# jamornsriwasansak/evplp

Measured on AMD Instinct MI355X. Metric: Mpaths/s, higher is better.
Workload: dtype f32

## Files before the change

evplp_amd/csrc/device_common.hpp:

```cpp
#pragma once
#include "evplp_types.h"
#include "ev_math.h"

namespace evplp {

#define EV_PI 3.14159265358979323846f
#define EV_INV_PI 0.318309886183790671537767526745028724068919291480912897495f
#define EV_DEV __device__ __forceinline__

struct V3 { float x, y, z; };
EV_DEV V3 v3(float x, float y, float z) { V3 r; r.x = x; r.y = y; r.z = z; return r; }
EV_DEV V3 v3(const float *p) { return v3(p[0], p[1], p[2]); }
EV_DEV V3 v3(float4 a) { return v3(a.x, a.y, a.z); }
EV_DEV V3 operator+(V3 a, V3 b) { return v3(a.x + b.x, a.y + b.y, a.z + b.z); }
EV_DEV V3 operator-(V3 a, V3 b) { return v3(a.x - b.x, a.y - b.y, a.z - b.z); }
EV_DEV V3 operator-(V3 a) { return v3(-a.x, -a.y, -a.z); }
EV_DEV V3 operator*(V3 a, V3 b) { return v3(a.x * b.x, a.y * b.y, a.z * b.z); }
EV_DEV V3 operator*(V3 a, float s) { return v3(a.x * s, a.y * s, a.z * s); }
EV_DEV V3 operator/(V3 a, float s) { return v3(a.x / s, a.y / s, a.z / s); }
EV_DEV float dot(V3 a, V3 b) { return a.x * b.x + a.y * b.y + a.z * b.z; }
EV_DEV V3 cross(V3 a, V3 b) { return v3(a.y * b.z - a.z * b.y, a.z * b.x - a.x * b.z, a.x * b.y - a.y * b.x); }
EV_DEV V3 normalize(V3 v) { float inv = 1.0f / sqrtf(dot(v, v)); return v * inv; }
EV_DEV V3 reflect(V3 i, V3 n) { float d = dot(n, i); return i - (n * 2.0f) * d; }
EV_DEV V3 faceforward(V3 n, V3 i, V3 nref) { return n * copysignf(1.0f, dot(i, nref)); }
// ... 203 lines not shown
    V3 p = v3(sin_t * cp, sin_t * sp, cos_t);
    Onb o = onb_make(r);
    out = onb_inverse(o, p);
    float unsafe_cos = dot(out, normal);
    float cos_n = fmaxf(unsafe_cos, 0.f);
    float cos_r = fmaxf(dot(out, r), 0.f);
    if (unsafe_cos > 0.0f) pdfw = (e + 1.0f) * 0.5f * evm_powf(cos_r, e) * EV_INV_PI;
    else pdfw = 0.0f;
    return rho_s * ((e + 2.0f) / (e + 1.0f) * cos_n);
}

EV_DEV V3 light_sample(const SceneDev &sc, V3 &position, V3 &normal, float &pdf, Rng &rng) {
    float r = rng_uniform(rng);
    uint32_t count = (uint32_t)sc.light_count, first = 0;
    while (count > 0) {
        uint32_t it = first, step = count / 2; it += step;
        if (sc.light_cdf[it] < r) { first = ++it; count -= step + 1; } else count = step;
    }
    if (first >= (uint32_t)sc.light_count) first = (uint32_t)sc.light_count - 1;
    const TriAttr &ta = sc.attrs[sc.light_first + (int32_t)first];
    float x = rng_uniform(rng);
    float y = rng_uniform(rng);
    float sq = sqrtf(x), beta = sq * (1.0f - y), gamma = sq * y;
    V3 p1 = v3(ta.v), p2 = v3(ta.v + 3), p3 = v3(ta.v + 6);
    position = p1 * beta + p2 * gamma + p3 * (1.0f - gamma - beta);
    normal = normalize(cross(p2 - p1, p3 - p1));
    pdf = 1.f / sc.light_area;
    return v3(sc.light_intensity) * sc.light_area;
}

EV_DEV bool slab_hit(const float *lo, const float *hi, V3 inv, V3 noi, float tmin, float tmax) {
    float t0x = __builtin_fmaf(lo[0], inv.x, noi.x), t1x = __builtin_fmaf(hi[0], inv.x, noi.x);
    float t0y = __builtin_fmaf(lo[1], inv.y, noi.y), t1y = __builtin_fmaf(hi[1], inv.y, noi.y);
    float t0z = __builtin_fmaf(lo[2], inv.z, noi.z), t1z = __builtin_fmaf(hi[2], inv.z, noi.z);
    float tn = fmaxf(fmaxf(fminf(t0x, t1x), fminf(t0y, t1y)), fmaxf(fminf(t0z, t1z), tmin));
    float tf = fminf(fminf(fmaxf(t0x, t1x), fmaxf(t0y, t1y)), fminf(fmaxf(t0z, t1z), tmax));
    return tn <= tf;
}
EV_DEV float slab_near(const float *lo, const float *hi, V3 inv, V3 noi, float tmin, float tmax, bool &hit) {
    float t0x = __builtin_fmaf(lo[0], inv.x, noi.x), t1x = __builtin_fmaf(hi[0], inv.x, noi.x);
    float t0y = __builtin_fmaf(lo[1], inv.y, noi.y), t1y = __builtin_fmaf(hi[1], inv.y, noi.y);
    float t0z = __builtin_fmaf(lo[2], inv.z, noi.z), t1z = __builtin_fmaf(hi[2], inv.z, noi.z);
    float tn = fmaxf(fmaxf(fminf(t0x, t1x), fminf(t0y, t1y)), fmaxf(fminf(t0z, t1z), tmin));
    float tf = fminf(fminf(fmaxf(t0x, t1x), fmaxf(t0y, t1y)), fminf(fmaxf(t0z, t1z), tmax));
    hit = tn <= tf;
    return tn;
}
EV_DEV float safe_rcp(float d) {
    float a = fabsf(d) < 1e-30f ? copysignf(1e-30f, d) : d;
    return __builtin_amdgcn_rcpf(a);
}

typedef int v16i __attribute__((ext_vector_type(16)));
typedef int v8i __attribute__((ext_vector_type(8)));
EV_DEV v16i sload16(const void *base, uint32_t byte_offset) {
    v16i r;
    asm("s_load_dwordx16 %0, %1, %2\n\ts_waitcnt lgkmcnt(0)" : "=&s"(r) : "s"(base), "s"(byte_offset));
    return r;
}
EV_DEV v8i sload8(const void *base, uint32_t byte_offset) {
    v8i r;
    asm("s_load_dwordx8 %0, %1, %2\n\ts_waitcnt lgkmcnt(0)" : "=&s"(r) : "s"(base), "s"(byte_offset));
    return r;
}
EV_DEV void sload16x2(const void *base, uint32_t byte_offset, v16i &a, v16i &b) {
    asm("s_load_dwordx16 %0, %2, %3\n\ts_load_dwordx16 %1, %2, %3 offset:0x40\n\ts_waitcnt lgkmcnt(0)" : "=&s"(a), "=&s"(b) : "s"(base), "s"(byte_offset));
}
EV_DEV void sload16x3(const void *base, uint32_t byte_offset, v16i &a, v16i &b, v16i &c) {
    asm("s_load_dwordx16 %0, %3, %4\n\ts_load_dwordx16 %1, %3, %4 offset:0x40\n\ts_load_dwordx16 %2, %3, %4 offset:0x80\n\ts_waitcnt lgkmcnt(0)"
        : "=&s"(a), "=&s"(b), "=&s"(c) : "s"(base), "s"(byte_offset));
}
template <class T> EV_DEV const T *pinned(const T *p) { asm("" : "+s"(p)); return p; }
#ifndef EVPLP_RING_NT
#define EVPLP_RING_NT 1
#endif
EV_DEV void lds_dma16(const void *gsrc, uint32_t lds_dst) {
    unsigned keep;
#if EVPLP_RING_NT
    asm volatile("s_mov_b32 %0, m0\n\ts_mov_b32 m0, %2\n\ts_nop 0\n\tglobal_load_lds_dwordx4 %1, off nt\n\ts_mov_b32 m0, %0" : "=&s"(keep) : "v"(gsrc), "s"(lds_dst) : "memory");
#else
    asm volatile("s_mov_b32 %0, m0\n\ts_mov_b32 m0, %2\n\ts_nop 0\n\tglobal_load_lds_dwordx4 %1, off\n\ts_mov_b32 m0, %0" : "=&s"(keep) : "v"(gsrc), "s"(lds_dst) : "memory");
#endif
}
EV_DEV void wait_vmcnt0() { asm volatile("s_waitcnt vmcnt(0)" ::: "memory"); }
template <int N> EV_DEV void wait_vmcnt() { asm volatile("s_waitcnt vmcnt(%0)" ::"n"(N) : "memory"); }
template <class T> EV_DEV uint32_t lds_offset(const T *p) { return (uint32_t)(uintptr_t)p; }
EV_DEV float f_of(int x) { return __int_as_float(x); }
EV_DEV v2f pk(int a, int b) { v2f r; r.x = __int_as_float(a); r.y = __int_as_float(b); return r; }
EV_DEV v2f bc(float a) { v2f r; r.x = a; r.y = a; return r; }
EV_DEV v2f pk_fma(v2f a, v2f b, v2f c) { return __builtin_elementwise_fma(a, b, c); }
EV_DEV v2f pk_min(v2f a, v2f b) { return __builtin_elementwise_min(a, b); }
EV_DEV v2f pk_max(v2f a, v2f b) { return __builtin_elementwise_max(a, b); }

EV_DEV v2f rcp_exact2(v2f x) {
#pragma clang fp contract(off)
    v2f r; r.x = __builtin_amdgcn_rcpf(x.x); r.y = __builtin_amdgcn_rcpf(x.y);
    const v2f one = bc(1.0f);
    const v2f e = pk_fma(-x, r, one);
    r = pk_fma(e, r, r);
    const v2f err = pk_fma(-x, r, one);
    return pk_fma(err, r, r);
}
EV_DEV unsigned long long ballot64(bool p) { return __builtin_amdgcn_ballot_w64(p); }
struct Hit2 { bool a, b; };
EV_DEV Hit2 tri_pair_test(v2f p0x, v2f p0y, v2f p0z, v2f e0x, v2f e0y, v2f e0z, v2f e1x, v2f e1y, v2f e1z, v2f nx, v2f ny, v2f nz,
                          V3 o, V3 d, float tmin, float tmax) {
#pragma clang fp contract(off)
    const v2f dx = bc(d.x), dy = bc(d.y), dz = bc(d.z);
    v2f den = pk_fma(nz, dz, pk_fma(ny, dy, nx * dx));
    const v2f inv = rcp_exact2(den);
    v2f qx = (p0x - bc(o.x)) * inv, qy = (p0y - bc(o.y)) * inv, qz = (p0z - bc(o.z)) * inv;
    v2f ix = pk_fma(dy, qz, -(dz * qy)), iy = pk_fma(dz, qx, -(dx * qz)), iz = pk_fma(dx, qy, -(dy * qx));
    v2f beta = pk_fma(iz, e1z, pk_fma(iy, e1y, ix * e1x));
    v2f gamma = pk_fma(iz, e0z, pk_fma(iy, e0y, ix * e0x));
    v2f t = pk_fma(nz, qz, pk_fma(ny, qy, nx * qx));
    const v2f rest = bc(1.0f) - (beta + gamma);
    Hit2 h;
    h.a = (t.x < tmax) & (t.x > tmin) & (__builtin_fminf(__builtin_fminf(beta.x, gamma.x), rest.x) >= 0.0f);
    h.b = (t.y < tmax) & (t.y > tmin) & (__builtin_fminf(__builtin_fminf(beta.y, gamma.y), rest.y) >= 0.0f);
    return h;
}

struct PairOps { v2f p0x, p0y, p0z, e0x, e0y, e0z, e1x, e1y, e1z, nx, ny, nz; };
EV_DEV bool tri_pair_any(const PairOps &T, V3 o, V3 d, float tmin, float tmax, uint32_t *exact_runs = nullptr) {
    if (exact_runs) (*exact_runs)++;
    Hit2 h = tri_pair_test(T.p0x, T.p0y, T.p0z, T.e0x, T.e0y, T.e0z, T.e1x, T.e1y, T.e1z, T.nx, T.ny, T.nz, o, d, tmin, tmax);
    return h.a | h.b;
}
struct LeafOps { PairOps A, B; uint32_t cnt; };
EV_DEV LeafOps fetch_leaf(const char *leaf_base, uint32_t leafref) {
    const uint32_t id = ~leafref;
    LeafOps L; L.cnt = (id & 3u) + 1u;
    const uint32_t off = (id >> 2) * 192u;
    v16i a, b;
    if (L.cnt > 2u) {
        v16i c;
        sload16x3(leaf_base, off, a, b, c);
        L.B.p0x = pk(b[8], b[9]); L.B.p0y = pk(b[10], b[11]); L.B.p0z = pk(b[12], b[13]); L.B.e0x = pk(b[14], b[15]); L.B.e0y = pk(c[0], c[1]); L.B.e0z = pk(c[2], c[3]);
        L.B.e1x = pk(c[4], c[5]); L.B.e1y = pk(c[6], c[7]); L.B.e1z = pk(c[8], c[9]); L.B.nx = pk(c[10], c[11]); L.B.ny = pk(c[12], c[13]); L.B.nz = pk(c[14], c[15]);
    } else sload16x2(leaf_base, off, a, b);
    L.A.p0x = pk(a[0], a[1]); L.A.p0y = pk(a[2], a[3]); L.A.p0z = pk(a[4], a[5]); L.A.e0x = pk(a[6], a[7]); L.A.e0y = pk(a[8], a[9]); L.A.e0z = pk(a[10], a[11]);
    L.A.e1x = pk(a[12], a[13]); L.A.e1y = pk(a[14], a[15]); L.A.e1z = pk(b[0], b[1]); L.A.nx = pk(b[2], b[3]); L.A.ny = pk(b[4], b[5]); L.A.nz = pk(b[6], b[7]);
    return L;
}

EV_DEV PairOps fetch_leaf_a(const char *leaf_base, uint32_t off, v16i &b) {
    v16i a;
    sload16x2(leaf_base, off, a, b);
    PairOps A;
    A.p0x = pk(a[0], a[1]); A.p0y = pk(a[2], a[3]); A.p0z = pk(a[4], a[5]); A.e0x = pk(a[6], a[7]); A.e0y = pk(a[8], a[9]); A.e0z = pk(a[10], a[11]);
    A.e1x = pk(a[12], a[13]); A.e1y = pk(a[14], a[15]); A.e1z = pk(b[0], b[1]); A.nx = pk(b[2], b[3]); A.ny = pk(b[4], b[5]); A.nz = pk(b[6], b[7]);
    return A;
}
EV_DEV PairOps fetch_leaf_b(const char *leaf_base, uint32_t off, const v16i &b) {
    const v16i c = sload16(leaf_base, off + 128u);
    PairOps B;
    B.p0x = pk(b[8], b[9]); B.p0y = pk(b[10], b[11]); B.p0z = pk(b[12], b[13]); B.e0x = pk(b[14], b[15]); B.e0y = pk(c[0], c[1]); B.e0z = pk(c[2], c[3]);
    B.e1x = pk(c[4], c[5]); B.e1y = pk(c[6], c[7]); B.e1z = pk(c[8], c[9]); B.nx = pk(c[10], c[11]); B.ny = pk(c[12], c[13]); B.nz = pk(c[14], c[15]);
    return B;
}

EV_DEV int lane_write(int value, int slot, int old) { return ((int)(threadIdx.x & 63u) == slot) ? value : old; }
EV_DEV int lane_read(int v, int slot) { return __builtin_amdgcn_readlane(v, slot); }

EV_DEV float clamp01(float x) { return __builtin_amdgcn_fmed3f(x, 0.0f, 1.0f); }

#ifndef EVPLP_TRAVERSAL_STATS
#define EVPLP_TRAVERSAL_STATS 0
#endif
struct WalkStats { uint32_t nodes, leaves, pairs, exact; int32_t hit_leaf; uint32_t syn; };

#ifndef EVPLP_WALK_ASM
#define EVPLP_WALK_ASM 1
#endif
#define EV_WALK_VISIT_ASM(T0, T1, T2, T3, T4, T5, T0L, T0H, T1L, T1H, T2L, T2H, T3L, T3H, T4L, T4H, T5L, T5H) EV_WALK_VISIT_ASM_("s", T0, T1, T2, T3, T4, T5, T0L, T0H, T1L, T1H, T2L, T2H, T3L, T3H, T4L, T4H, T5L, T5H)
#define EV_WALK_VISIT_ASM_(NC, T0, T1, T2, T3, T4, T5, T0L, T0H, T1L, T1H, T2L, T2H, T3L, T3H, T4L, T4H, T5L, T5H)                               \
    asm volatile(                                                                                                                            \
        "v_pk_fma_f32 " T0 ", %[cx], %[pa], %[pd] op_sel:[0,0,0] op_sel_hi:[1,0,0]\n\t"                                                                                     \
        "v_pk_fma_f32 " T1 ", %[cy], %[pa], %[pd] op_sel:[0,1,1] op_sel_hi:[1,1,1]\n\t"                                                                                     \
        "v_pk_fma_f32 " T2 ", %[cz], %[pb], %[pe] op_sel:[0,0,0] op_sel_hi:[1,0,0]\n\t"                                                                                     \
        "v_pk_fma_f32 " T3 ", %[hx], %[pb], " T0 " op_sel:[0,1,0] op_sel_hi:[1,1,1] neg_lo:[0,1,0] neg_hi:[0,1,0]\n\t"                                                        \
        "v_pk_fma_f32 " T4 ", %[hy], %[pc], " T1 " op_sel:[0,0,0] op_sel_hi:[1,0,1] neg_lo:[0,1,0] neg_hi:[0,1,0]\n\t"                                                        \
        "v_pk_fma_f32 " T5 ", %[hz], %[pc], " T2 " op_sel:[0,1,0] op_sel_hi:[1,1,1] neg_lo:[0,1,0] neg_hi:[0,1,0]\n\t"                                                        \
        "v_pk_fma_f32 " T0 ", %[hx], %[pb], " T0 " op_sel:[0,1,0] op_sel_hi:[1,1,1]\n\t"                                                                                     \
        "v_pk_fma_f32 " T1 ", %[hy], %[pc], " T1 " op_sel:[0,0,0] op_sel_hi:[1,0,1]\n\t"                                                                                     \
        "v_pk_fma_f32 " T2 ", %[hz], %[pc], " T2 " op_sel:[0,1,0] op_sel_hi:[1,1,1]\n\t"                                                                                     \
        "v_max3_f32 " T3L ", " T3L ", " T4L ", " T5L " clamp\n\t"                                                                            \
        "v_min3_f32 " T0L ", " T0L ", " T1L ", " T2L " clamp\n\t"                                                                            \
        "v_max3_f32 " T3H ", " T3H ", " T4H ", " T5H " clamp\n\t"                                                                            \
        "v_min3_f32 " T0H ", " T0H ", " T1H ", " T2H " clamp\n\t"                                                                            \
        "v_cmp_lt_f32 vcc, " T3L ", " T0L "\n\t"                                                                                             \
        "v_cmp_lt_f32 %[m1], " T3H ", " T0H "\n\t"                                                                                           \
        "s_or_b64 %[t64], vcc, %[m1]\n\t"                                                                                                    \
        "s_cbranch_scc0 L_pop%=\n\t"                                                                                                         \
        "s_cmp_eq_u64 vcc, 0\n\t"                                                                                                            \
        "s_cbranch_scc1 L_c1%=\n\t"                                                                                                          \
        "s_cmp_eq_u64 %[m1], 0\n\t"                                                                                                          \
        "s_cbranch_scc1 L_c0%=\n\t"                                                                                                          \
        "s_bcnt1_i32_b64 %[p0], vcc\n\t"                                                                                                     \
        "s_bcnt1_i32_b64 %[p1], %[m1]\n\t"                                                                                                   \
        "s_cmp_ge_i32 %[p0], %[p1]\n\t"                                                                                                      \
        "s_cselect_b32 %[p0], %[c1], %[c0]\n\t"                                                                                              \
        "s_cselect_b32 %[cur], %[c0], %[c1]\n\t"                                                                                             \
        "s_mov_b32 m0, %[sp]\n\t"                                                                                                            \
        "s_add_i32 %[sp], %[sp], 1\n\t"                                                                                                      \
        "v_writelane_b32 %[vstack], %[p0], m0\n\t"                                                                                           \
        "s_branch L_end%=\n"                                                                                                                 \
        "L_c0%=:\n\t"                                                                                                                        \
        "s_mov_b32 %[cur], %[c0]\n\t"                                                                                                        \
        "s_branch L_end%=\n"                                                                                                                 \
        "L_c1%=:\n\t"                                                                                                                        \
        "s_mov_b32 %[cur], %[c1]\n\t"                                                                                                        \
        "s_branch L_end%=\n"                                                                                                                 \
        "L_pop%=:\n\t"                                                                                                                       \
        "s_brev_b32 %[cur], 1\n\t"                                                                                                           \
        "s_cmp_eq_u32 %[sp], 0\n\t"                                                                                                          \
        "s_cbranch_scc1 L_end%=\n\t"                                                                                                         \
        "s_sub_i32 %[sp], %[sp], 1\n\t"                                                                                                      \
        "s_nop 0\n\t"                                                                                                                        \
        "v_readlane_b32 %[cur], %[vstack], %[sp]\n"                                                                                          \
        "L_end%=:\n"                                                                                                                         \
        : [cur] "+s"(cur), [sp] "+s"(sp), [vstack] "+v"(vstack), [m1] "=&s"(m1_), [t64] "=&s"(t64_), [p0] "=&s"(p0_), [p1] "=&s"(p1_)          \
        : [cx] NC(cx_), [cy] NC(cy_), [cz] NC(cz_), [hx] NC(hx_), [hy] NC(hy_), [hz] NC(hz_), [c0] "s"(c0_), [c1] "s"(c1_),              \
          [pa] "v"(pa_), [pb] "v"(pb_), [pc] "v"(pc_),                                     \
          [pd] "v"(pd_), [pe] "v"(pe_), [lane] "v"(lane_id)                                                                 \
        : "vcc", "scc", "m0", T0L, T0H, T1L, T1H, T2L, T2H, T3L, T3H, T4L, T4H, T5L, T5H)

template <int VT = 0, bool CUT = false>
EV_DEV bool occluded_wave(const char *node_base, const char *leaf_base, V3 o, V3 d, float tmin, float tmax, bool alive_lane, WalkStats *ws = nullptr, const char *cut = nullptr, uint32_t cut_off = 0u,
                          const float4 *cut_lds = nullptr) {
    unsigned long long alive = ballot64(alive_lane), hitm = 0ull;
    if (alive == 0ull) return false;
    uint32_t cut_end = 0u;
    constexpr bool kCutLds = CUT && VT != 0 && EVPLP_WALK_ASM && !EVPLP_TRAVERSAL_STATS;
    if constexpr (kCutLds) {
        const int32_t nsyn = __builtin_amdgcn_readfirstlane(__float_as_int(cut_lds[3].z));
        if (nsyn == 0) return false;
        cut_off = 0u; cut_end = (uint32_t)nsyn;
    } else if constexpr (CUT) {
        int32_t nsyn;
        asm volatile("s_load_dword %0, %1, %2 offset:0x38\n\ts_waitcnt lgkmcnt(0)" : "=s"(nsyn) : "s"(cut), "s"(cut_off) : "memory");
        if (nsyn == 0) return false;
        cut_end = cut_off + ((uint32_t)nsyn << 6);
    }
    const V3 inv0 = v3(safe_rcp(d.x), safe_rcp(d.y), safe_rcp(d.z));
    const float ku = 1.0f / (tmax - tmin);
    const V3 inv = inv0 * ku;
    const v2f ivx = bc(inv.x), ivy = bc(inv.y), ivz = bc(inv.z);
    const v2f avx = bc(fabsf(inv.x)), avy = bc(fabsf(inv.y)), avz = bc(fabsf(inv.z));
    const float dead = __builtin_inff();
    v2f nox = bc(alive_lane ? (-(o.x * inv0.x) - tmin) * ku : dead), noy = bc(alive_lane ? (-(o.y * inv0.y) - tmin) * ku : dead),
        noz = bc(alive_lane ? (-(o.z * inv0.z) - tmin) * ku : dead);
    int sp = 0;
    int vstack = 0;
    int32_t cur = 0;
#if EVPLP_WALK_ASM && !EVPLP_TRAVERSAL_STATS
    if constexpr (VT != 0) {
        static_assert(VT == 52 || VT == 116, "reserved temporaries: v[52:63] or v[116:127]");
        const int lane_id = (int)(threadIdx.x & 63u);
        v2f pa_, pb_, pc_, pd_, pe_;
        pa_.x = ivx.x; pa_.y = ivy.x; pb_.x = ivz.x; pb_.y = avx.x; pc_.x = avy.x; pc_.y = avz.x;
        pd_.x = nox.x; pd_.y = noy.x; pe_.x = noz.x; pe_.y = noz.x;
#define EV_VISIT(N)                                                                                                                          \
        {                                                                                                                                    \
            const v2f cx_ = pk(N[0], N[1]), cy_ = pk(N[2], N[3]), cz_ = pk(N[4], N[5]), hx_ = pk(N[6], N[7]), hy_ = pk(N[8], N[9]), hz_ = pk(N[10], N[11]); \
            const int32_t c0_ = N[12], c1_ = N[13];                                                                                          \
            unsigned long long m1_, t64_; int32_t p0_, p1_;                                                                                  \
            if constexpr (VT == 52) EV_WALK_VISIT_ASM("v[52:53]", "v[54:55]", "v[56:57]", "v[58:59]", "v[60:61]", "v[62:63]", "v52", "v53", "v54", "v55", "v56", "v57", "v58", "v59", "v60", "v61", "v62", "v63"); \
            else EV_WALK_VISIT_ASM("v[116:117]", "v[118:119]", "v[120:121]", "v[122:123]", "v[124:125]", "v[126:127]", "v116", "v117", "v118", "v119", "v120", "v121", "v122", "v123", "v124", "v125", "v126", "v127"); \
        }
        for (;;) {
            if constexpr (CUT) {
                if (cut_off >= cut_end) break;
                v16i syn;
                {
                    const float4 *q = cut_lds + 4u * cut_off;
#pragma unroll
                    for (int w = 0; w < 4; w++) {
                        const float4 qq = q[w];
                        if (w < 3 || true) { syn[4 * w] = __builtin_amdgcn_readfirstlane(__float_as_int(qq.x)); syn[4 * w + 1] = __builtin_amdgcn_readfirstlane(__float_as_int(qq.y)); }
                        if (w < 3) { syn[4 * w + 2] = __builtin_amdgcn_readfirstlane(__float_as_int(qq.z)); syn[4 * w + 3] = __builtin_amdgcn_readfirstlane(__float_as_int(qq.w)); }
                    }
                    syn[14] = 0; syn[15] = 0;
                }
                cut_off++;
                EV_VISIT(syn)
            }
            for (;;) {
                while (cur >= 0) {
                    const v16i n = sload16(node_base, (uint32_t)cur << 6);
                    EV_VISIT(n)
                }
                if (cur == kNoChild) break;
                const uint32_t cnt = (((uint32_t)~cur) & 3u) + 1u, loff = (((uint32_t)~cur) >> 2) * 192u;
                bool any;
                if constexpr (CUT) {
                    v16i lb;
                    { const PairOps A = fetch_leaf_a(leaf_base, loff, lb); any = tri_pair_any(A, o, d, tmin, tmax); }
                    if (cnt > 2u) { const PairOps B = fetch_leaf_b(leaf_base, loff, lb); any = any | tri_pair_any(B, o, d, tmin, tmax); }
                } else {
                    const LeafOps L = fetch_leaf(leaf_base, (uint32_t)cur);
                    any = tri_pair_any(L.A, o, d, tmin, tmax);
                    if (cnt > 2u) any = any | tri_pair_any(L.B, o, d, tmin, tmax);
                }
                const unsigned long long hm = ballot64(any) & alive;
                if (hm != 0ull) {
                    hitm |= hm;
                    alive &= ~hm;
                    if (alive == 0ull) return ((hitm >> (threadIdx.x & 63u)) & 1ull) != 0ull;
                    if (any) { pd_ = bc(dead); pe_ = bc(dead); }
                }
                if (sp == 0) break;
                sp--;
                cur = lane_read(vstack, sp);
            }
            if constexpr (!CUT) break;
        }
#undef EV_VISIT
        return ((hitm >> (threadIdx.x & 63u)) & 1ull) != 0ull;
    }
#endif
    auto visit_cpp = [&](const v16i &n) {
        const v2f ax = pk_fma(pk(n[0], n[1]), ivx, nox), ay = pk_fma(pk(n[2], n[3]), ivy, noy), az = pk_fma(pk(n[4], n[5]), ivz, noz);
        const v2f hx = pk(n[6], n[7]), hy = pk(n[8], n[9]), hz = pk(n[10], n[11]);
        const v2f enx = pk_fma(hx, -avx, ax), eny = pk_fma(hy, -avy, ay), enz = pk_fma(hz, -avz, az);
        const v2f exx = pk_fma(hx, avx, ax), exy = pk_fma(hy, avy, ay), exz = pk_fma(hz, avz, az);
        const float tn0 = clamp01(fmaxf(fmaxf(enx.x, eny.x), enz.x)), tf0 = clamp01(fminf(fminf(exx.x, exy.x), exz.x));
        const float tn1 = clamp01(fmaxf(fmaxf(enx.y, eny.y), enz.y)), tf1 = clamp01(fminf(fminf(exx.y, exy.y), exz.y));
        const unsigned long long m0 = ballot64(tn0 < tf0), m1 = ballot64(tn1 < tf1);
        const int32_t c0 = n[12], c1 = n[13];
        const uint32_t a0 = (uint32_t)m0 | (uint32_t)(m0 >> 32), a1 = (uint32_t)m1 | (uint32_t)(m1 >> 32);
        if ((a0 | a1) == 0u) { if (sp == 0) cur = kNoChild; else { sp--; cur = lane_read(vstack, sp); } return; }
        if (a0 == 0u) { cur = c1; return; }
        if (a1 == 0u) { cur = c0; return; }
        int p0, p1;
        asm("s_bcnt1_i32_b64 %0, %1" : "=s"(p0) : "s"(m0) : "scc");
        asm("s_bcnt1_i32_b64 %0, %1" : "=s"(p1) : "s"(m1) : "scc");
        const bool first0 = p0 >= p1;
        const int32_t oth = first0 ? c1 : c0;
        vstack = lane_write(oth, sp, vstack);
        sp++;
        cur = first0 ? c0 : c1;
    };
    for (;;) {
        if constexpr (CUT) {
            if (cut_off >= cut_end) break;
            const v16i syn = sload16(cut, cut_off);
            cut_off += 64u;
#if EVPLP_TRAVERSAL_STATS
            if (ws) { ws->nodes++; ws->syn++; }
#endif
            visit_cpp(syn);
        }
        for (;;) {
            while (cur >= 0) {
                const v16i n = sload16(node_base, (uint32_t)cur << 6);
#if EVPLP_TRAVERSAL_STATS
                if (ws) ws->nodes++;
#endif
                visit_cpp(n);
            }
            if (cur == kNoChild) break;
            {
                const uint32_t id = (uint32_t)~cur;
                const uint32_t cnt = (id & 3u) + 1u;
                const LeafOps L = fetch_leaf(leaf_base, (uint32_t)cur);
#if EVPLP_TRAVERSAL_STATS
                if (ws) { ws->leaves++; ws->pairs += cnt > 2u ? 2u : 1u; }
                uint32_t *ex = ws ? &ws->exact : nullptr;
// ... 374 lines not shown
```

evplp_amd/csrc/kernels_gather.hip:

```cpp
#include "device_common.hpp"
#include "kernels.h"
#include <algorithm>

namespace evplp {

constexpr int kRecF4 = sizeof(evplp_record) / 16;

struct Pixel {
    V3 p1, n1, rd, rs; float e; V3 wi10;
};

struct Vpl {
    V3 pos, n, flux, fdir, rd, rs; float psel, e;
};
EV_DEV Vpl load_vpl(const float4 *r) {
    Vpl v; float4 a = r[0], b = r[1], c = r[2], d = r[3], e = r[4], f = r[5];
    v.pos = v3(a); v.n = v3(b); v.psel = b.w; v.flux = v3(c); v.fdir = v3(d); v.rd = v3(e); v.rs = v3(f); v.e = f.w;
    return v;
}

EV_DEV float phong_eval_f_hw(V3 out, V3 in, V3 n, float e) {
    V3 r = reflect(-in, n);
    float d = fmaxf(dot(out, r), 0.0f);
    if (d <= 0.000001f) return 0.0f;
// ... 95 lines not shown
    const int x = ix.tx * 8 + (lane & 7), ly = ix.ty * 8 + (lane >> 3);
    return (uint32_t)max(min(ly, st.local_rows - 1), 0) * (uint32_t)st.W + (uint32_t)min(x, st.W - 1);
}

EV_DEV uint32_t item_cut_group(const GatherArgs &a, const Item &t) {
    const int tx = __builtin_amdgcn_readfirstlane(t.x) >> 3, ty = __builtin_amdgcn_readfirstlane(t.ly) >> 3;
    return (uint32_t)(((ty >> a.cut_gh_log2) - a.cut_group_row_first) * a.cut_groups_x + (tx >> a.cut_gw_log2));
}

#ifndef EVPLP_CUT_RING
#define EVPLP_CUT_RING 3
#endif
#ifndef EVPLP_PX_LDS
#define EVPLP_PX_LDS 1
#endif
constexpr int kGatherPxFloats = 64 * (EVPLP_PX_LDS ? 10 : 3);
#ifndef EVPLP_GATHER_WAVES
#define EVPLP_GATHER_WAVES 8
#endif

EV_DEV Vpl fetch_vpl(const evplp_record *r) {
    const v16i ra = *reinterpret_cast<const v16i *>(r);
    const v8i rb = *reinterpret_cast<const v8i *>(reinterpret_cast<const int *>(r) + 16);
    Vpl v;
    v.pos = v3(f_of(ra[0]), f_of(ra[1]), f_of(ra[2])); v.n = v3(f_of(ra[4]), f_of(ra[5]), f_of(ra[6])); v.psel = f_of(ra[7]);
    v.flux = v3(f_of(ra[8]), f_of(ra[9]), f_of(ra[10])); v.fdir = v3(f_of(ra[12]), f_of(ra[13]), f_of(ra[14]));
    v.rd = v3(f_of(rb[0]), f_of(rb[1]), f_of(rb[2])); v.rs = v3(f_of(rb[4]), f_of(rb[5]), f_of(rb[6])); v.e = f_of(rb[7]);
    return v;
}
EV_DEV void fetch_vpl_head(const evplp_record *vpls, uint32_t i, V3 &pos, V3 &n, float &psel) {
    const v8i ra = sload8(vpls, i * (uint32_t)sizeof(evplp_record));
    pos = v3(f_of(ra[0]), f_of(ra[1]), f_of(ra[2])); n = v3(f_of(ra[4]), f_of(ra[5]), f_of(ra[6])); psel = f_of(ra[7]);
}
EV_DEV void fetch_vpl_tail(const evplp_record *vpls, uint32_t i, Vpl &v) {
    const v16i rb = sload16(vpls, i * (uint32_t)sizeof(evplp_record) + 32u);
    v.flux = v3(f_of(rb[0]), f_of(rb[1]), f_of(rb[2])); v.fdir = v3(f_of(rb[4]), f_of(rb[5]), f_of(rb[6]));
    v.rd = v3(f_of(rb[8]), f_of(rb[9]), f_of(rb[10])); v.rs = v3(f_of(rb[12]), f_of(rb[13]), f_of(rb[14])); v.e = f_of(rb[15]);
}

#if EVPLP_GATHER_TIMES
__device__ unsigned long long g_gather_times[2 * 131072];
extern "C" int evplp_debug_gather_times(unsigned long long *out, int n) { return (int)hipMemcpyFromSymbol(out, HIP_SYMBOL(g_gather_times), sizeof(unsigned long long) * (size_t)n); }
#endif
EV_DEV void item_cost_add(const GatherArgs &a, int ty, unsigned long long t0, int waves) {
    const unsigned long long dt = __builtin_amdgcn_s_memrealtime() - t0;
    if (threadIdx.x == 0) atomicAdd(&a.block_cost[(ty * 8) / a.st.strip_rows], dt * 8ull / (unsigned long long)waves);
}
template <bool CUT, bool COST = false>
#if EVPLP_WALK_ASM && !EVPLP_TRAVERSAL_STATS
__attribute__((amdgpu_num_vgpr(52)))
#endif
__global__ __launch_bounds__(64, EVPLP_GATHER_WAVES) void gather_vpl_kernel(GatherArgs a) {
    unsigned long long t_cost = 0ull;
    if constexpr (COST) t_cost = __builtin_amdgcn_s_memrealtime();
#if EVPLP_GATHER_TIMES
    const unsigned long long t_start = __builtin_amdgcn_s_memrealtime();
#endif
    extern __shared__ float s_dyn[];
    float *const s_wi10 = s_dyn, *const s_lvl = s_dyn + kGatherPxFloats;
    const int lane = threadIdx.x;
    const Item t = item_setup(a, lane, (int)blockIdx.x);
    if (!t.has_tile) return;
    const uint32_t p = t.p;

    Pixel px;
    float4 gp = a.g_pos[p], gn = a.g_nrm[p], gd = a.g_dif[p], gs = a.g_phg[p];
    px.p1 = v3(gp); px.n1 = v3(gn); px.rd = v3(gd); px.rs = v3(gs); px.e = gs.w;
#ifndef EVPLP_WI10_LDS
#define EVPLP_WI10_LDS 1
#endif
    {
        const V3 w = normalize(v3(a.fp.camera_pos) - px.p1);
        s_wi10[lane] = w.x; s_wi10[64 + lane] = w.y; s_wi10[128 + lane] = w.z;
        px.wi10 = EVPLP_WI10_LDS ? v3(0.f, 0.f, 0.f) : w;
    }
    bool px_glossy = true;
    if constexpr (EVPLP_PX_LDS != 0) {
        static_assert(EVPLP_WI10_LDS != 0, "EVPLP_PX_LDS continues the LDS column of the view direction");
        s_wi10[192 + lane] = px.rd.x; s_wi10[256 + lane] = px.rd.y; s_wi10[320 + lane] = px.rd.z;
        s_wi10[384 + lane] = px.rs.x; s_wi10[448 + lane] = px.rs.y; s_wi10[512 + lane] = px.rs.z; s_wi10[576 + lane] = px.e;
        px_glossy = ballot64(px.rs.x != 0.0f || px.rs.y != 0.0f || px.rs.z != 0.0f) != 0ull;
        px.rd = v3(0.f, 0.f, 0.f); px.rs = v3(0.f, 0.f, 0.f); px.e = 0.0f;
    }
    const bool valid = t.in_image && gp.w != 0.0f;

    const uint32_t nvpl = *a.nvpl;
    const int k = a.splits_per_wave;
    const char *node_base = pinned(reinterpret_cast<const char *>(a.sc.nodes)), *leaf_base = pinned(reinterpret_cast<const char *>(a.sc.leaves));
    const evplp_record *vpls = pinned(a.vpls);
    const char *cuts_g = nullptr;
    if constexpr (CUT) cuts_g = pinned(a.cuts + (size_t)item_cut_group(a, t) * a.cut_vpl_stride * (size_t)kCutSlotBytes);
    V3 total = v3(0.f, 0.f, 0.f);
    uint32_t rays = t.in_image ? 0x80000000u : 0u, shaded = 0;
#if EVPLP_TRAVERSAL_STATS
    int32_t cache_leaf = kNoChild; bool prev_all_occ = false;
#endif
    constexpr bool kRing = CUT && EVPLP_WALK_ASM && !EVPLP_TRAVERSAL_STATS;
    constexpr int kRingSlots = EVPLP_CUT_RING, kAhead = kRingSlots - 1;
    __shared__ float4 s_cut[kRing ? kRingSlots : 1][kCutSlotBytes / 16];
    int pj = 0; uint32_t pi = (uint32_t)(t.group * k), qslot = 0u;
    auto ring_skip_empty = [&]() { while (pj < k && pi >= nvpl) { pj++; pi = (uint32_t)(t.group * k + pj); } };
    auto ring_issue = [&](uint32_t slot) {
        if (lane < kCutSlotBytes / 16) lds_dma16(cuts_g + (size_t)pi * kCutSlotBytes + (size_t)lane * 16u, lds_offset(&s_cut[slot][0]));
        pi += (uint32_t)kVplSplit; ring_skip_empty();
    };
    if constexpr (kRing) {
        ring_skip_empty();
        for (int q = 0; q < kAhead; q++) if (pj < k) ring_issue((uint32_t)q);
    }
    for (int jj = 0; jj < k; jj++) {
        const uint32_t split = (uint32_t)(t.group * k + jj);
        V3 result = v3(0.f, 0.f, 0.f);
        for (uint32_t i = split; i < nvpl; i += kVplSplit) {
            const float4 *cut_lds = nullptr;
            if constexpr (kRing) {
                if (pj < k) { ring_issue((qslot + (uint32_t)kAhead) % (uint32_t)kRingSlots); wait_vmcnt<kAhead>(); }
                else wait_vmcnt0();
                cut_lds = &s_cut[qslot][0];
                qslot = (qslot + 1u) % (uint32_t)kRingSlots;
            }
            V3 vpos, vn; float vpsel; fetch_vpl_head(vpls, i, vpos, vn, vpsel);
            V3 v12 = vpos - px.p1;
            float c1 = fmaxf(dot_exact(px.n1, v12), 0.0f);
            float c2 = fmaxf(-dot_exact(vn, v12), 0.0f);
            float c1c2 = c1 * c2;
            bool active = valid && !(c1c2 <= 0.0f);
            if (ballot64(active) == 0ull) continue;
            rays += active ? 1u : 0u;
            bool occ;
            {
#if EVPLP_TRAVERSAL_STATS
                unsigned long long cache_kill = 0ull;
                const unsigned long long act_m = ballot64(active);
                if (cache_leaf != kNoChild) {
                    const LeafOps L = fetch_leaf(leaf_base, (uint32_t)cache_leaf);
                    const V3 dd = -v12;
                    bool any = tri_pair_any(L.A, vpos, dd, 0.0001f, 1.0f - 0.0001f);
                    if (L.cnt > 2u) any = any | tri_pair_any(L.B, vpos, dd, 0.0001f, 1.0f - 0.0001f);
                    cache_kill = ballot64(any) & act_m;
                }
                WalkStats ws = { 0u, 0u, 0u, 0u, kNoChild, 0u };
                occ = occluded_wave<0, CUT>(node_base, leaf_base, vpos, -v12, 0.0001f, 1.0f - 0.0001f, active, &ws, cuts_g, i * (uint32_t)kCutSlotBytes);
                const bool all_occ = ballot64(active && !occ) == 0ull;
                const unsigned long long occ_m = ballot64(active && occ);
                if (lane == 0) {
                    atomicAdd(&a.counters->hist[41], (unsigned long long)__builtin_popcountll(occ_m));
                    atomicAdd(&a.counters->nodes, (unsigned long long)ws.nodes);
                    atomicAdd(&a.counters->aux, (unsigned long long)ws.syn);
                    atomicAdd(&a.counters->hist[min(ws.leaves, 31u)], 1ull);
                    atomicAdd(&a.counters->hist[32], 1ull);
                    atomicAdd(&a.counters->hist[33], (unsigned long long)ws.pairs);
                    if (all_occ) { atomicAdd(&a.counters->hist[34], 1ull); atomicAdd(&a.counters->hist[36], (unsigned long long)ws.nodes); atomicAdd(&a.counters->hist[37], (unsigned long long)ws.leaves); }
                    if (ws.leaves == 0u) atomicAdd(&a.counters->hist[35], (unsigned long long)ws.nodes);
                    if (cache_leaf != kNoChild) {
                        atomicAdd(&a.counters->hist[42], 1ull);
                        atomicAdd(&a.counters->hist[40], (unsigned long long)__builtin_popcountll(cache_kill));
                        if (cache_kill == act_m) { atomicAdd(&a.counters->hist[38], 1ull); atomicAdd(&a.counters->hist[39], (unsigned long long)ws.nodes); }
                        if (prev_all_occ) { atomicAdd(&a.counters->hist[44], 1ull); if (cache_kill == act_m) atomicAdd(&a.counters->hist[43], 1ull); }
                    }
                    atomicAdd(&a.counters->hist[45 + min(ws.nodes / 16u, 18u)], 1ull);
                }
                if (ws.hit_leaf != kNoChild) cache_leaf = ws.hit_leaf;
                prev_all_occ = all_occ;
#else
                occ = occluded_wave<EVPLP_WALK_ASM ? 52 : 0, CUT>(node_base, leaf_base, vpos, -v12, 0.0001f, 1.0f - 0.0001f, active, nullptr, cuts_g, i * (uint32_t)kCutSlotBytes, cut_lds);
#endif
            }
            const bool lit = active && !occ;
            if (ballot64(lit) == 0ull) continue;
            Vpl v; fetch_vpl_head(vpls, i, v.pos, v.n, v.psel); fetch_vpl_tail(vpls, i, v);
            evplp_frame_params fps; float pdf_mc2;
            {
                const void *ka = (const void *)__builtin_amdgcn_kernarg_segment_ptr();
                typedef int v4i_ __attribute__((ext_vector_type(4)));
                v4i_ q; int q2;
                asm volatile("s_load_dwordx4 %0, %2, %3\n\ts_load_dword %1, %2, %4\n\ts_waitcnt lgkmcnt(0)" : "=&s"(q), "=&s"(q2)
                             : "s"(ka), "s"((uint32_t)(offsetof(GatherArgs, fp) + offsetof(evplp_frame_params, mis_mode))), "s"((uint32_t)offsetof(GatherArgs, pdf_mc2)) : "memory");
                fps.mis_mode = (uint32_t)q[0]; fps.pdf_mc = f_of(q[1]); fps.clamping_value = f_of(q[2]); pdf_mc2 = f_of(q2);
            }
            if (lit) { result = result + vpl_shade<EVPLP_PX_LDS != 0>(fps, pdf_mc2, px, v, v12, c1c2, EVPLP_WI10_LDS ? s_wi10 + lane : nullptr, px_glossy); shaded++; }
        }
        {
            int lev = 0;
            while ((jj >> lev) & 1) {
                float *q = s_lvl + lev * 192 + lane;
                result = v3(q[0], q[64], q[128]) + result;
                lev++;
            }
            float *q = s_lvl + lev * 192 + lane;
            q[0] = result.x; q[64] = result.y; q[128] = result.z;
        }
        total = result;
    }
#if EVPLP_DEBUG_NAN
    if ((rays >> 31) != 0u && !(isfinite(total.x) && isfinite(total.y) && isfinite(total.z))) atomicAdd(&a.counters->nonfinite, 1ull);
#endif
#if EVPLP_XCD_TIMES
    if (lane == 0) atomicMax(&a.counters->hist[16 + (blockIdx.x & 7u)], (unsigned long long)__builtin_amdgcn_s_memrealtime());
#endif
#if EVPLP_GATHER_TIMES
    if (lane == 0 && (blockIdx.x & 15u) == 0u && (blockIdx.x >> 4) < 131072u) { g_gather_times[2 * (blockIdx.x >> 4)] = t_start; g_gather_times[2 * (blockIdx.x >> 4) + 1] = __builtin_amdgcn_s_memrealtime(); }
#endif
    int lane_out = lane, blk_out = (int)blockIdx.x;
    asm volatile("" : "+v"(lane_out), "+s"(blk_out));
    const bool in_image = (rays >> 31) != 0u;
    rays &= 0xffffu;
    if (in_image) a.partial[(size_t)item_index(a, blk_out).sg * a.partial_stride + item_texel(a, lane_out, blk_out)] = make_float4(total.x, total.y, total.z, __uint_as_float(rays | (shaded << 16)));
    if constexpr (COST) item_cost_add(a, item_index(a, blk_out).ty, t_cost, EVPLP_GATHER_WAVES);
}

__global__ __launch_bounds__(256) void gather_reduce_kernel(GatherArgs a, int stencil_test) {
    const size_t i = (size_t)blockIdx.x * 256 + threadIdx.x;
    const size_t n = (size_t)a.st.W * a.st.local_rows;
    unsigned long long rays = 0ull, shaded = 0ull;
    bool writes = i < n;
    if (writes) {
        const int ly = (int)(i / a.st.W);
        if (a.st.global_row(ly) >= a.st.H) writes = false;
        else if (stencil_test && a.g_pos[i].w == 0.0f) writes = false;
    }
    if (writes) {
        const int groups = kVplSplit / a.splits_per_wave;
        V3 r = v3(0.f, 0.f, 0.f), lv0 = r, lv1 = r, lv2 = r, lv3 = r, lv4 = r, lv5 = r, lv6 = r;
        for (int g = 0; g < groups; g++) {
            float4 q = a.partial[(size_t)g * a.partial_stride + i];
            const uint32_t st = __float_as_uint(q.w);
            rays += st & 0xffffu; shaded += st >> 16;
            r = v3(q.x, q.y, q.z);
#define EV_MERGE(L, NEXT) if (((g >> L) & 1) == 0) lv##L = r; else { r = lv##L + r; NEXT }
            EV_MERGE(0, EV_MERGE(1, EV_MERGE(2, EV_MERGE(3, EV_MERGE(4, EV_MERGE(5, EV_MERGE(6, ;)))))))
#undef EV_MERGE
        }
        const float inv = (float)a.fp.num_vpl_light_paths, acc = (float)a.fp.do_accumulate;
        float4 old = a.out[i];
        a.out[i] = make_float4(r.x / inv + acc * old.x, r.y / inv + acc * old.y, r.z / inv + acc * old.z, 0.0f + acc * old.w);
    }
    __shared__ unsigned long long s_sum[2];
    if (threadIdx.x < 2) s_sum[threadIdx.x] = 0ull;
    __syncthreads();
    for (int off = 32; off > 0; off >>= 1) { rays += __shfl_down(rays, off); shaded += __shfl_down(shaded, off); }
    if ((threadIdx.x & 63) == 0) { atomicAdd(&s_sum[0], rays); atomicAdd(&s_sum[1], shaded); }
    __syncthreads();
    if (threadIdx.x == 0) {
        const int shard = blockIdx.x & (kCounterShards - 1);
        atomicAdd(&a.counters->shard_rays[shard], s_sum[0]);
        atomicAdd(&a.counters->shard_shaded[shard], s_sum[1]);
    }
}

#ifndef EVPLP_LVC_WIDE
#define EVPLP_LVC_WIDE 0
// ... 480 lines not shown
```

Before: 42500.

## Fuse LDS cut-node reads into walk asm and trim per-lane state

The cut-node visit now reads the node from LDS with ds_read_b128 inside the inline asm and uses readfirstlane only for the two child indices. The packed slab math then runs directly on the loaded VGPRs, which avoids 14 readfirstlane conversions and the SGPR staging per visited node. The ring DMA issue masks exec to the low 16 lanes inside asm instead of branching on the lane index. The 'valid' flag is replaced by writing NaN into px.p1.x so that invalid pixels fail the c1c2 test, freeing a mask register. The NaN trick relies on dot_exact propagating NaN, and the hard-coded VGPR choices risk register clobbers.

```diff
diff --git a/evplp_amd/csrc/device_common.hpp b/evplp_amd/csrc/device_common.hpp
--- a/evplp_amd/csrc/device_common.hpp
+++ b/evplp_amd/csrc/device_common.hpp
@@ -309,6 +309,16 @@
     asm volatile("s_mov_b32 %0, m0\n\ts_mov_b32 m0, %2\n\ts_nop 0\n\tglobal_load_lds_dwordx4 %1, off\n\ts_mov_b32 m0, %0" : "=&s"(keep) : "v"(gsrc), "s"(lds_dst) : "memory");
 #endif
 }
+EV_DEV void lds_dma16_lo16(const void *gsrc, uint32_t lds_dst) {
+    unsigned keep; unsigned long long keep_exec;
+    asm volatile("s_mov_b32 %0, m0\n\ts_mov_b64 %1, exec\n\ts_and_b32 exec_lo, exec_lo, 0xffff\n\ts_mov_b32 exec_hi, 0\n\ts_mov_b32 m0, %3\n\ts_nop 0\n\t"
+#if EVPLP_RING_NT
+                 "global_load_lds_dwordx4 %2, off nt\n\t"
+#else
+                 "global_load_lds_dwordx4 %2, off\n\t"
+#endif
+                 "s_mov_b64 exec, %1\n\ts_mov_b32 m0, %0" : "=&s"(keep), "=&s"(keep_exec) : "v"(gsrc), "s"(lds_dst) : "memory", "scc");
+}
 EV_DEV void wait_vmcnt0() { asm volatile("s_waitcnt vmcnt(0)" ::: "memory"); }
 template <int N> EV_DEV void wait_vmcnt() { asm volatile("s_waitcnt vmcnt(%0)" ::"n"(N) : "memory"); }
 template <class T> EV_DEV uint32_t lds_offset(const T *p) { return (uint32_t)(uintptr_t)p; }
@@ -400,24 +410,7 @@
 #ifndef EVPLP_WALK_ASM
 #define EVPLP_WALK_ASM 1
 #endif
-#define EV_WALK_VISIT_ASM(T0, T1, T2, T3, T4, T5, T0L, T0H, T1L, T1H, T2L, T2H, T3L, T3H, T4L, T4H, T5L, T5H) EV_WALK_VISIT_ASM_("s", T0, T1, T2, T3, T4, T5, T0L, T0H, T1L, T1H, T2L, T2H, T3L, T3H, T4L, T4H, T5L, T5H)
-#define EV_WALK_VISIT_ASM_(NC, T0, T1, T2, T3, T4, T5, T0L, T0H, T1L, T1H, T2L, T2H, T3L, T3H, T4L, T4H, T5L, T5H)                               \
-    asm volatile(                                                                                                                            \
-        "v_pk_fma_f32 " T0 ", %[cx], %[pa], %[pd] op_sel:[0,0,0] op_sel_hi:[1,0,0]\n\t"                                                                                     \
-        "v_pk_fma_f32 " T1 ", %[cy], %[pa], %[pd] op_sel:[0,1,1] op_sel_hi:[1,1,1]\n\t"                                                                                     \
-        "v_pk_fma_f32 " T2 ", %[cz], %[pb], %[pe] op_sel:[0,0,0] op_sel_hi:[1,0,0]\n\t"                                                                                     \
-        "v_pk_fma_f32 " T3 ", %[hx], %[pb], " T0 " op_sel:[0,1,0] op_sel_hi:[1,1,1] neg_lo:[0,1,0] neg_hi:[0,1,0]\n\t"                                                        \
-        "v_pk_fma_f32 " T4 ", %[hy], %[pc], " T1 " op_sel:[0,0,0] op_sel_hi:[1,0,1] neg_lo:[0,1,0] neg_hi:[0,1,0]\n\t"                                                        \
-        "v_pk_fma_f32 " T5 ", %[hz], %[pc], " T2 " op_sel:[0,1,0] op_sel_hi:[1,1,1] neg_lo:[0,1,0] neg_hi:[0,1,0]\n\t"                                                        \
-        "v_pk_fma_f32 " T0 ", %[hx], %[pb], " T0 " op_sel:[0,1,0] op_sel_hi:[1,1,1]\n\t"                                                                                     \
-        "v_pk_fma_f32 " T1 ", %[hy], %[pc], " T1 " op_sel:[0,0,0] op_sel_hi:[1,0,1]\n\t"                                                                                     \
-        "v_pk_fma_f32 " T2 ", %[hz], %[pc], " T2 " op_sel:[0,1,0] op_sel_hi:[1,1,1]\n\t"                                                                                     \
-        "v_max3_f32 " T3L ", " T3L ", " T4L ", " T5L " clamp\n\t"                                                                            \
-        "v_min3_f32 " T0L ", " T0L ", " T1L ", " T2L " clamp\n\t"                                                                            \
-        "v_max3_f32 " T3H ", " T3H ", " T4H ", " T5H " clamp\n\t"                                                                            \
-        "v_min3_f32 " T0H ", " T0H ", " T1H ", " T2H " clamp\n\t"                                                                            \
-        "v_cmp_lt_f32 vcc, " T3L ", " T0L "\n\t"                                                                                             \
-        "v_cmp_lt_f32 %[m1], " T3H ", " T0H "\n\t"                                                                                           \
+#define EV_WALK_DECIDE_ASM_                                                                                                          \
         "s_or_b64 %[t64], vcc, %[m1]\n\t"                                                                                                    \
         "s_cbranch_scc0 L_pop%=\n\t"                                                                                                         \
         "s_cmp_eq_u64 vcc, 0\n\t"                                                                                                            \
@@ -446,12 +439,63 @@
         "s_sub_i32 %[sp], %[sp], 1\n\t"                                                                                                      \
         "s_nop 0\n\t"                                                                                                                        \
         "v_readlane_b32 %[cur], %[vstack], %[sp]\n"                                                                                          \
-        "L_end%=:\n"                                                                                                                         \
+        "L_end%=:\n"
+#define EV_WALK_VISIT_ASM(T0, T1, T2, T3, T4, T5, T0L, T0H, T1L, T1H, T2L, T2H, T3L, T3H, T4L, T4H, T5L, T5H) EV_WALK_VISIT_ASM_("s", T0, T1, T2, T3, T4, T5, T0L, T0H, T1L, T1H, T2L, T2H, T3L, T3H, T4L, T4H, T5L, T5H)
+#define EV_WALK_VISIT_ASM_(NC, T0, T1, T2, T3, T4, T5, T0L, T0H, T1L, T1H, T2L, T2H, T3L, T3H, T4L, T4H, T5L, T5H)                               \
+    asm volatile(                                                                                                                            \
+        "v_pk_fma_f32 " T0 ", %[cx], %[pa], %[pd] op_sel:[0,0,0] op_sel_hi:[1,0,0]\n\t"                                                                                     \
+        "v_pk_fma_f32 " T1 ", %[cy], %[pa], %[pd] op_sel:[0,1,1] op_sel_hi:[1,1,1]\n\t"                                                                                     \
+        "v_pk_fma_f32 " T2 ", %[cz], %[pb], %[pe] op_sel:[0,0,0] op_sel_hi:[1,0,0]\n\t"                                                                                     \
+        "v_pk_fma_f32 " T3 ", %[hx], %[pb], " T0 " op_sel:[0,1,0] op_sel_hi:[1,1,1] neg_lo:[0,1,0] neg_hi:[0,1,0]\n\t"                                                        \
+        "v_pk_fma_f32 " T4 ", %[hy], %[pc], " T1 " op_sel:[0,0,0] op_sel_hi:[1,0,1] neg_lo:[0,1,0] neg_hi:[0,1,0]\n\t"                                                        \
+        "v_pk_fma_f32 " T5 ", %[hz], %[pc], " T2 " op_sel:[0,1,0] op_sel_hi:[1,1,1] neg_lo:[0,1,0] neg_hi:[0,1,0]\n\t"                                                        \
+        "v_pk_fma_f32 " T0 ", %[hx], %[pb], " T0 " op_sel:[0,1,0] op_sel_hi:[1,1,1]\n\t"                                                                                     \
+        "v_pk_fma_f32 " T1 ", %[hy], %[pc], " T1 " op_sel:[0,0,0] op_sel_hi:[1,0,1]\n\t"                                                                                     \
+        "v_pk_fma_f32 " T2 ", %[hz], %[pc], " T2 " op_sel:[0,1,0] op_sel_hi:[1,1,1]\n\t"                                                                                     \
+        "v_max3_f32 " T3L ", " T3L ", " T4L ", " T5L " clamp\n\t"                                                                            \
+        "v_min3_f32 " T0L ", " T0L ", " T1L ", " T2L " clamp\n\t"                                                                            \
+        "v_max3_f32 " T3H ", " T3H ", " T4H ", " T5H " clamp\n\t"                                                                            \
+        "v_min3_f32 " T0H ", " T0H ", " T1H ", " T2H " clamp\n\t"                                                                            \
+        "v_cmp_lt_f32 vcc, " T3L ", " T0L "\n\t"                                                                                             \
+        "v_cmp_lt_f32 %[m1], " T3H ", " T0H "\n\t"                                                                                           \
+        EV_WALK_DECIDE_ASM_                                                                                                                  \
         : [cur] "+s"(cur), [sp] "+s"(sp), [vstack] "+v"(vstack), [m1] "=&s"(m1_), [t64] "=&s"(t64_), [p0] "=&s"(p0_), [p1] "=&s"(p1_)          \
         : [cx] NC(cx_), [cy] NC(cy_), [cz] NC(cz_), [hx] NC(hx_), [hy] NC(hy_), [hz] NC(hz_), [c0] "s"(c0_), [c1] "s"(c1_),              \
           [pa] "v"(pa_), [pb] "v"(pb_), [pc] "v"(pc_),                                     \
           [pd] "v"(pd_), [pe] "v"(pe_), [lane] "v"(lane_id)                                                                 \
         : "vcc", "scc", "m0", T0L, T0H, T1L, T1H, T2L, T2H, T3L, T3H, T4L, T4H, T5L, T5H)
+
+#define EV_WALK_VISIT_LDS_ASM_(Q0, Q1, Q2, T0, T1, T2, T3, T4, T5, T0L, T0H, T1L, T1H, T2L, T2H, T3L, T3H, T4L, T4H, T5L, T5H)                   \
+    asm volatile(                                                                                                                            \
+        "ds_read_b128 " Q0 ", %[addr]\n\t"                                                                                                   \
+        "ds_read_b128 " Q1 ", %[addr] offset:16\n\t"                                                                                         \
+        "ds_read_b128 " Q2 ", %[addr] offset:32\n\t"                                                                                         \
+        "ds_read_b32 %[k0], %[addr] offset:48\n\t"                                                                                           \
+        "ds_read_b32 %[k1], %[addr] offset:52\n\t"                                                                                           \
+        "s_waitcnt lgkmcnt(0)\n\t"                                                                                                           \
+        "v_pk_fma_f32 " T0 ", " T0 ", %[pa], %[pd] op_sel:[0,0,0] op_sel_hi:[1,0,0]\n\t"                                                     \
+        "v_pk_fma_f32 " T1 ", " T1 ", %[pa], %[pd] op_sel:[0,1,1] op_sel_hi:[1,1,1]\n\t"                                                     \
+        "v_pk_fma_f32 " T2 ", " T2 ", %[pb], %[pe] op_sel:[0,0,0] op_sel_hi:[1,0,0]\n\t"                                                     \
+        "v_readfirstlane_b32 %[c0], %[k0]\n\t"                                                                                               \
+        "v_readfirstlane_b32 %[c1], %[k1]\n\t"                                                                                               \
+        "v_pk_fma_f32 %[e], " T3 ", %[pb], " T0 " op_sel:[0,1,0] op_sel_hi:[1,1,1] neg_lo:[0,1,0] neg_hi:[0,1,0]\n\t"                        \
+        "v_pk_fma_f32 " T0 ", " T3 ", %[pb], " T0 " op_sel:[0,1,0] op_sel_hi:[1,1,1]\n\t"                                                    \
+        "v_pk_fma_f32 " T3 ", " T4 ", %[pc], " T1 " op_sel:[0,0,0] op_sel_hi:[1,0,1] neg_lo:[0,1,0] neg_hi:[0,1,0]\n\t"                      \
+        "v_pk_fma_f32 " T1 ", " T4 ", %[pc], " T1 " op_sel:[0,0,0] op_sel_hi:[1,0,1]\n\t"                                                    \
+        "v_pk_fma_f32 " T4 ", " T5 ", %[pc], " T2 " op_sel:[0,1,0] op_sel_hi:[1,1,1] neg_lo:[0,1,0] neg_hi:[0,1,0]\n\t"                      \
+        "v_pk_fma_f32 " T2 ", " T5 ", %[pc], " T2 " op_sel:[0,1,0] op_sel_hi:[1,1,1]\n\t"                                                    \
+        "v_pk_mov_b32 " T5 ", %[e], %[e] op_sel:[0,1]\n\t"                                                                                   \
+        "v_min3_f32 " T0L ", " T0L ", " T1L ", " T2L " clamp\n\t"                                                                            \
+        "v_max3_f32 " T5L ", " T5L ", " T3L ", " T4L " clamp\n\t"                                                                            \
+        "v_min3_f32 " T0H ", " T0H ", " T1H ", " T2H " clamp\n\t"                                                                            \
+        "v_max3_f32 " T5H ", " T5H ", " T3H ", " T4H " clamp\n\t"                                                                            \
+        "v_cmp_lt_f32 vcc, " T5L ", " T0L "\n\t"                                                                                             \
+        "v_cmp_lt_f32 %[m1], " T5H ", " T0H "\n\t"                                                                                           \
+        EV_WALK_DECIDE_ASM_                                                                                                                  \
+        : [cur] "+s"(cur), [sp] "+s"(sp), [vstack] "+v"(vstack), [m1] "=&s"(m1_), [t64] "=&s"(t64_), [p0] "=&s"(p0_), [p1] "=&s"(p1_),         \
+          [c0] "=&s"(c0_), [c1] "=&s"(c1_), [k0] "=&v"(k0_), [k1] "=&v"(k1_), [e] "=&v"(e_)                                                  \
+        : [addr] "v"(addr_), [pa] "v"(pa_), [pb] "v"(pb_), [pc] "v"(pc_), [pd] "v"(pd_), [pe] "v"(pe_)                                       \
+        : "vcc", "scc", "m0", "memory", T0L, T0H, T1L, T1H, T2L, T2H, T3L, T3H, T4L, T4H, T5L, T5H)
 
 template <int VT = 0, bool CUT = false>
 EV_DEV bool occluded_wave(const char *node_base, const char *leaf_base, V3 o, V3 d, float tmin, float tmax, bool alive_lane, WalkStats *ws = nullptr, const char *cut = nullptr, uint32_t cut_off = 0u,
@@ -499,19 +543,13 @@
         for (;;) {
             if constexpr (CUT) {
                 if (cut_off >= cut_end) break;
-                v16i syn;
-                {
-                    const float4 *q = cut_lds + 4u * cut_off;
-#pragma unroll
-                    for (int w = 0; w < 4; w++) {
-                        const float4 qq = q[w];
-                        if (w < 3 || true) { syn[4 * w] = __builtin_amdgcn_readfirstlane(__float_as_int(qq.x)); syn[4 * w + 1] = __builtin_amdgcn_readfirstlane(__float_as_int(qq.y)); }
-                        if (w < 3) { syn[4 * w + 2] = __builtin_amdgcn_readfirstlane(__float_as_int(qq.z)); syn[4 * w + 3] = __builtin_amdgcn_readfirstlane(__float_as_int(qq.w)); }
-                    }
-                    syn[14] = 0; syn[15] = 0;
-                }
+                const uint32_t addr_ = lds_offset(cut_lds + 4u * cut_off);
                 cut_off++;
-                EV_VISIT(syn)
+                unsigned long long m1_, t64_; int32_t p0_, p1_, c0_, c1_, k0_, k1_; v2f e_;
+                if constexpr (VT == 52) EV_WALK_VISIT_LDS_ASM_("v[52:55]", "v[56:59]", "v[60:63]", "v[52:53]", "v[54:55]", "v[56:57]", "v[58:59]", "v[60:61]", "v[62:63]",
+                                                               "v52", "v53", "v54", "v55", "v56", "v57", "v58", "v59", "v60", "v61", "v62", "v63");
+                else EV_WALK_VISIT_LDS_ASM_("v[116:119]", "v[120:123]", "v[124:127]", "v[116:117]", "v[118:119]", "v[120:121]", "v[122:123]", "v[124:125]", "v[126:127]",
+                                            "v116", "v117", "v118", "v119", "v120", "v121", "v122", "v123", "v124", "v125", "v126", "v127");
             }
             for (;;) {
                 while (cur >= 0) {
diff --git a/evplp_amd/csrc/kernels_gather.hip b/evplp_amd/csrc/kernels_gather.hip
--- a/evplp_amd/csrc/kernels_gather.hip
+++ b/evplp_amd/csrc/kernels_gather.hip
@@ -201,7 +201,7 @@
         px_glossy = ballot64(px.rs.x != 0.0f || px.rs.y != 0.0f || px.rs.z != 0.0f) != 0ull;
         px.rd = v3(0.f, 0.f, 0.f); px.rs = v3(0.f, 0.f, 0.f); px.e = 0.0f;
     }
-    const bool valid = t.in_image && gp.w != 0.0f;
+    if (!(t.in_image && gp.w != 0.0f)) px.p1.x = __builtin_nanf("");
 
     const uint32_t nvpl = *a.nvpl;
     const int k = a.splits_per_wave;
@@ -220,7 +220,8 @@
     int pj = 0; uint32_t pi = (uint32_t)(t.group * k), qslot = 0u;
     auto ring_skip_empty = [&]() { while (pj < k && pi >= nvpl) { pj++; pi = (uint32_t)(t.group * k + pj); } };
     auto ring_issue = [&](uint32_t slot) {
-        if (lane < kCutSlotBytes / 16) lds_dma16(cuts_g + (size_t)pi * kCutSlotBytes + (size_t)lane * 16u, lds_offset(&s_cut[slot][0]));
+        static_assert(kCutSlotBytes == 16 * 16, "one slot = 16 lanes x 16 bytes");
+        lds_dma16_lo16(cuts_g + (size_t)pi * kCutSlotBytes + (size_t)lane * 16u, lds_offset(&s_cut[slot][0]));
         pi += (uint32_t)kVplSplit; ring_skip_empty();
     };
     if constexpr (kRing) {
@@ -243,7 +244,7 @@
             float c1 = fmaxf(dot_exact(px.n1, v12), 0.0f);
             float c2 = fmaxf(-dot_exact(vn, v12), 0.0f);
             float c1c2 = c1 * c2;
-            bool active = valid && !(c1c2 <= 0.0f);
+            bool active = !(c1c2 <= 0.0f);
             if (ballot64(active) == 0ull) continue;
             rays += active ? 1u : 0u;
             bool occ;
@@ -285,7 +286,8 @@
                 occ = occluded_wave<EVPLP_WALK_ASM ? 52 : 0, CUT>(node_base, leaf_base, vpos, -v12, 0.0001f, 1.0f - 0.0001f, active, nullptr, cuts_g, i * (uint32_t)kCutSlotBytes, cut_lds);
 #endif
             }
-            const bool lit = active && !occ;
+            asm volatile("" : "+v"(c1c2));
+            const bool lit = !(c1c2 <= 0.0f) && !occ;
             if (ballot64(lit) == 0ull) continue;
             Vpl v; fetch_vpl_head(vpls, i, v.pos, v.n, v.psel); fetch_vpl_tail(vpls, i, v);
             evplp_frame_params fps; float pdf_mc2;
```

New measurement: 42910, median of 6. No clear change (+1.0%).
